# achraf-15/neural_image_compression

Hardware: AMD Instinct MI355X
Metric: images/sec (256x256 RGB, batch 32) fwd+bwd (higher is better)
Workload: dtype f32; 1 GPU; cfg2: JointAutoregressiveHierarchical(M=192,K=1) fwd+rd_loss(lambda=0.01)+bwd+Adam, 32x3x256x256 per GPU, fp32; global_batch=32, parallelism=dp1, step=eager (autograd)

## Files before the change

neural_image_compression_amd/csrc/lic_gdn.hip:

```cpp
#include "lic_common.h"
#include <stdlib.h>

namespace {

constexpr int GD_BM = 64;
constexpr int GD_BK = 16;

struct GdnParams {
  const float* x;
  const float* g;
  const float* norm;
  const float* w;
  const float* beta;
  const float* res;
  float* out;
  float* out2;
  float* cs_t;
  float* cs_dx;
  long P;
  int inverse;
};

template <int TN, int MODE>
__global__ __launch_bounds__(256) void gdn_kernel(const GdnParams p) {
  constexpr int C = 64 * TN;
  constexpr int LDX = C + 4;
  constexpr int NCH = C / GD_BK;
  constexpr int SLOTS = GD_BM * C / 4 / 256;
  __shared__ __attribute__((aligned(16))) float smem[GD_BM * LDX];
  const int tid = threadIdx.x, lane = tid & 63;
  const int wave = __builtin_amdgcn_readfirstlane(tid >> 6);
  const int wm0 = (wave >> 1) * 32, wn0 = (wave & 1) * (32 * TN);
  const int li = lane & 31, lh = lane >> 5;
  const long m0 = (long)blockIdx.x * GD_BM;
  const bool inv = p.inverse != 0;

  if (MODE == 0) {
    f32x4 a[SLOTS];
#pragma unroll
    for (int u = 0; u < SLOTS; ++u) {
      const int idx = u * 256 + tid;
      const int row = idx / (C / 4), c4 = (idx - row * (C / 4)) * 4;
      const bool ok = m0 + row < p.P;
      a[u] = *reinterpret_cast<const f32x4*>(p.x + (ok ? (m0 + row) * C + c4 : 0L));
      if (!ok) a[u] = f32x4{0.f, 0.f, 0.f, 0.f};
    }
#pragma unroll
    for (int u = 0; u < SLOTS; ++u) {
      const int idx = u * 256 + tid;
      const int row = idx / (C / 4), c4 = (idx - row * (C / 4)) * 4;
      *reinterpret_cast<f32x4*>(&smem[row * LDX + c4]) = a[u];
    }
  } else {
#pragma unroll
  for (int s0 = 0; s0 < SLOTS; s0 += 4) {
    f32x4 a[4], b[4], c[4];
    bool ok[4];
#pragma unroll
    for (int u = 0; u < 4; ++u) {
      const int idx = (s0 + u) * 256 + tid;
      const int row = idx / (C / 4), c4 = (idx - row * (C / 4)) * 4;
      ok[u] = m0 + row < p.P;
      const long off = ok[u] ? (m0 + row) * C + c4 : 0L;
      a[u] = *reinterpret_cast<const f32x4*>(p.x + off);
      b[u] = *reinterpret_cast<const f32x4*>(p.g + off);
      c[u] = *reinterpret_cast<const f32x4*>(p.norm + off);
    }
#pragma unroll
    for (int u = 0; u < 4; ++u) {
      const int idx = (s0 + u) * 256 + tid;
      const int row = idx / (C / 4), c4 = (idx - row * (C / 4)) * 4;
      f32x4 v;
#pragma unroll
      for (int e = 0; e < 4; ++e) {
        const float rs = __builtin_amdgcn_rsqf(c[u][e]);
        const float gx = b[u][e] * a[u][e];
        v[e] = inv ? 0.5f * gx * rs : -0.5f * gx * rs * (rs * rs);
      }
      if (ok[u]) *reinterpret_cast<f32x4*>(p.out2 + (m0 + row) * C + c4) = v;
      if (!ok[u]) v = f32x4{0.f, 0.f, 0.f, 0.f};
      *reinterpret_cast<f32x4*>(&smem[row * LDX + c4]) = v;
    }
  }
  }
  __syncthreads();
  if (MODE == 1 && p.cs_t && tid < C) {
    float a = 0.0f;
#pragma unroll 8
    for (int r = 0; r < GD_BM; ++r) a += smem[r * LDX + tid];
    p.cs_t[(long)blockIdx.x * C + tid] = a;
  }

  f32x16 acc[TN];
#pragma unroll
  for (int b = 0; b < TN; ++b)
#pragma unroll
    for (int r = 0; r < 16; ++r) acc[b][r] = 0.0f;
  const float* glane = p.w + ((long)(wn0 >> 5) * 512 + lane * 4);
  const float* xrow = smem + (wm0 + li) * LDX + lh * 8;
  f32x4 g0[TN][2], g1[TN][2];
  auto load_g = [&](f32x4 (&rg)[TN][2], int c) {
    const float* src = glane + (long)(c < NCH ? c : NCH - 1) * C * GD_BK;
#pragma unroll
    for (int b = 0; b < TN; ++b) {
      rg[b][0] = *reinterpret_cast<const f32x4*>(src + b * 512);
      rg[b][1] = *reinterpret_cast<const f32x4*>(src + b * 512 + 256);
    }
  };
  auto pool = [&](int c, const f32x4 (&rg)[TN][2]) {
    f32x4 a0 = *reinterpret_cast<const f32x4*>(xrow + c * GD_BK);
    f32x4 a1 = *reinterpret_cast<const f32x4*>(xrow + c * GD_BK + 4);
    if (MODE == 0) {
      a0 = a0 * a0;
      a1 = a1 * a1;
    }
#pragma unroll
    for (int t = 0; t < 8; ++t)
#pragma unroll
      for (int b = 0; b < TN; ++b)
        acc[b] = __builtin_amdgcn_mfma_f32_32x32x2f32((t < 4 ? a0 : a1)[t & 3], rg[b][t >> 2][t & 3], acc[b], 0, 0, 0);
  };
  load_g(g0, 0);
#pragma unroll 1
  for (int c = 0; c < NCH; c += 2) {
    load_g(g1, c + 1);
    pool(c, g0);
    load_g(g0, c + 2);
    pool(c + 1, g1);
  }

  __shared__ __attribute__((aligned(16))) float patch[MODE == 0 ? 4 : 1][MODE == 0 ? 1024 : 4];
  if (MODE == 1) __syncthreads();
  float* stg = MODE == 0 ? patch[wave] : smem + wave * 1024;
  const int c4 = (lane & 7) * 4, r8 = lane >> 3;
  f32x4 csum[TN];
#pragma unroll
  for (int b = 0; b < TN; ++b) csum[b] = f32x4{0.f, 0.f, 0.f, 0.f};
#pragma unroll
  for (int b = 0; b < TN; ++b) {
#pragma unroll
    for (int r = 0; r < 16; ++r) stg[((r & 3) + 8 * (r >> 2) + 4 * lh) * 32 + li] = acc[b][r];
    __builtin_amdgcn_wave_barrier();
    const int col = wn0 + b * 32 + c4;
#pragma unroll
    for (int it = 0; it < 4; ++it) {
      const int rr = it * 8 + r8;
      const long pix = m0 + wm0 + rr;
      if (pix >= p.P) continue;
      const f32x4 s4 = *reinterpret_cast<const f32x4*>(&stg[rr * 32 + c4]);
      const long off = pix * C + col;
      f32x4 o;
      if (MODE == 0) {
        const f32x4 n4 = s4 + *reinterpret_cast<const f32x4*>(p.beta + col);
        const f32x4 x4 = *reinterpret_cast<const f32x4*>(&smem[(wm0 + rr) * LDX + col]);
#pragma unroll
        for (int e = 0; e < 4; ++e)
          o[e] = x4[e] * (inv ? __builtin_amdgcn_sqrtf(n4[e]) : __builtin_amdgcn_rsqf(n4[e]));
        if (p.out2) *reinterpret_cast<f32x4*>(p.out2 + off) = n4;
        if (p.res) o += *reinterpret_cast<const f32x4*>(p.res + off);
      } else {
        const f32x4 n4 = *reinterpret_cast<const f32x4*>(p.norm + off);
        const f32x4 g4 = *reinterpret_cast<const f32x4*>(p.g + off);
        const f32x4 x4 = *reinterpret_cast<const f32x4*>(p.x + off);
#pragma unroll
        for (int e = 0; e < 4; ++e) {
          const float f = inv ? __builtin_amdgcn_sqrtf(n4[e]) : __builtin_amdgcn_rsqf(n4[e]);
          o[e] = g4[e] * f + 2.0f * x4[e] * s4[e];
        }
        csum[b] += o;
      }
      *reinterpret_cast<f32x4*>(p.out + off) = o;
    }
    __builtin_amdgcn_wave_barrier();
  }
  if (MODE == 1 && p.cs_dx) {
    __syncthreads();
    float* part = smem;
#pragma unroll
    for (int b = 0; b < TN; ++b)
      *reinterpret_cast<f32x4*>(&part[(((wave >> 1) * 8 + r8) * C) + wn0 + b * 32 + c4]) = csum[b];
    __syncthreads();
    if (tid < C) {
      float a = 0.0f;
#pragma unroll
      for (int k = 0; k < 16; ++k) a += part[k * C + tid];
      p.cs_dx[(long)blockIdx.x * C + tid] = a;
    }
  }
}

template <int TN>
__global__ __launch_bounds__(256, 2) void gdn_bwd_reg_kernel(const GdnParams p) {
  constexpr int C = 64 * TN;
  constexpr int LDX = C + 4;
  constexpr int NCH = C / GD_BK;
  __shared__ __attribute__((aligned(16))) float smem[GD_BM * LDX];
  const int tid = threadIdx.x, lane = tid & 63;
  const int wave = __builtin_amdgcn_readfirstlane(tid >> 6);
  const int wm0 = (wave >> 1) * 32, wn0 = (wave & 1) * (32 * TN);
  const int li = lane & 31, lh = lane >> 5;
  const int c4 = (lane & 7) * 4, r8 = lane >> 3;
  const long m0 = (long)blockIdx.x * GD_BM;
  const bool inv = p.inverse != 0;

  f32x4 u[TN][4], xx[TN][4];
#pragma unroll
  for (int b = 0; b < TN; ++b) {
    f32x4 gg[4], nn[4];
    bool ok[4];
#pragma unroll
    for (int it = 0; it < 4; ++it) {
      const long pix = m0 + wm0 + it * 8 + r8;
      ok[it] = pix < p.P;
      const long off = ok[it] ? pix * C + wn0 + b * 32 + c4 : 0L;
      xx[b][it] = *reinterpret_cast<const f32x4*>(p.x + off);
      gg[it] = *reinterpret_cast<const f32x4*>(p.g + off);
      nn[it] = *reinterpret_cast<const f32x4*>(p.norm + off);
    }
#pragma unroll
    for (int it = 0; it < 4; ++it) {
      const int row = wm0 + it * 8 + r8, col = wn0 + b * 32 + c4;
      f32x4 t;
#pragma unroll
      for (int e = 0; e < 4; ++e) {
        const float rs = __builtin_amdgcn_rsqf(nn[it][e]);
        const float gx = gg[it][e] * xx[b][it][e];
        t[e] = inv ? 0.5f * gx * rs : -0.5f * gx * rs * (rs * rs);
        u[b][it][e] = gg[it][e] * (inv ? __builtin_amdgcn_sqrtf(nn[it][e]) : rs);
      }
      if (ok[it]) {
        *reinterpret_cast<f32x4*>(p.out2 + (m0 + row) * C + col) = t;
      } else {
        t = f32x4{0.f, 0.f, 0.f, 0.f};
        u[b][it] = t;
        xx[b][it] = t;
      }
      *reinterpret_cast<f32x4*>(&smem[row * LDX + col]) = t;
    }
  }
  __syncthreads();
  if (p.cs_t && tid < C) {
    float a = 0.0f;
#pragma unroll 8
    for (int r = 0; r < GD_BM; ++r) a += smem[r * LDX + tid];
    p.cs_t[(long)blockIdx.x * C + tid] = a;
  }

  f32x16 acc[TN];
#pragma unroll
  for (int b = 0; b < TN; ++b)
#pragma unroll
    for (int r = 0; r < 16; ++r) acc[b][r] = 0.0f;
  const float* glane = p.w + ((long)(wn0 >> 5) * 512 + lane * 4);
  const float* xrow = smem + (wm0 + li) * LDX + lh * 8;
  f32x4 g0[TN][2], g1[TN][2];
  auto load_g = [&](f32x4 (&rg)[TN][2], int c) {
    const float* src = glane + (long)(c < NCH ? c : NCH - 1) * C * GD_BK;
#pragma unroll
    for (int b = 0; b < TN; ++b) {
      rg[b][0] = *reinterpret_cast<const f32x4*>(src + b * 512);
      rg[b][1] = *reinterpret_cast<const f32x4*>(src + b * 512 + 256);
    }
  };
  auto pool = [&](int c, const f32x4 (&rg)[TN][2]) {
    const f32x4 a0 = *reinterpret_cast<const f32x4*>(xrow + c * GD_BK);
    const f32x4 a1 = *reinterpret_cast<const f32x4*>(xrow + c * GD_BK + 4);
#pragma unroll
    for (int t = 0; t < 8; ++t)
#pragma unroll
      for (int b = 0; b < TN; ++b)
        acc[b] = __builtin_amdgcn_mfma_f32_32x32x2f32((t < 4 ? a0 : a1)[t & 3], rg[b][t >> 2][t & 3], acc[b], 0, 0, 0);
  };
  load_g(g0, 0);
#pragma unroll 1
  for (int c = 0; c < NCH; c += 2) {
    load_g(g1, c + 1);
    pool(c, g0);
    load_g(g0, c + 2);
    pool(c + 1, g1);
  }
  __syncthreads();
  float* stg = smem + wave * 1024;
  f32x4 csum[TN];
#pragma unroll
  for (int b = 0; b < TN; ++b) {
    csum[b] = f32x4{0.f, 0.f, 0.f, 0.f};
#pragma unroll
    for (int r = 0; r < 16; ++r) stg[((r & 3) + 8 * (r >> 2) + 4 * lh) * 32 + li] = acc[b][r];
    __builtin_amdgcn_wave_barrier();
#pragma unroll
    for (int it = 0; it < 4; ++it) {
      const int rr = it * 8 + r8;
      const long pix = m0 + wm0 + rr;
      if (pix >= p.P) continue;
      const f32x4 s4 = *reinterpret_cast<const f32x4*>(&stg[rr * 32 + c4]);
      f32x4 o;
#pragma unroll
      for (int e = 0; e < 4; ++e) o[e] = u[b][it][e] + 2.0f * xx[b][it][e] * s4[e];
      csum[b] += o;
      *reinterpret_cast<f32x4*>(p.out + pix * C + wn0 + b * 32 + c4) = o;
    }
    __builtin_amdgcn_wave_barrier();
  }
  if (p.cs_dx) {
    __syncthreads();
    float* part = smem;
#pragma unroll
    for (int b = 0; b < TN; ++b)
      *reinterpret_cast<f32x4*>(&part[(((wave >> 1) * 8 + r8) * C) + wn0 + b * 32 + c4]) = csum[b];
    __syncthreads();
    if (tid < C) {
      float a = 0.0f;
#pragma unroll
      for (int k = 0; k < 16; ++k) a += part[k * C + tid];
      p.cs_dx[(long)blockIdx.x * C + tid] = a;
    }
  }
}

bool gd_al16(const void* q) { return (reinterpret_cast<uintptr_t>(q) & 15) == 0; }

template <int MODE>
int gdn_launch(const GdnParams& p, int C, hipStream_t s) {
  const unsigned grid = (unsigned)cdiv64(p.P, GD_BM);
  if (C == 192)
    hipLaunchKernelGGL((gdn_kernel<3, MODE>), dim3(grid), dim3(256), 0, s, p);
  else if (C == 128)
    hipLaunchKernelGGL((gdn_kernel<2, MODE>), dim3(grid), dim3(256), 0, s, p);
  else
    hipLaunchKernelGGL((gdn_kernel<1, MODE>), dim3(grid), dim3(256), 0, s, p);
  return lic_check_launch();
}

}

LIC_EXPORT int lic_gdn_supported(int32_t C) { return C == 64 || C == 128 || C == 192; }

LIC_EXPORT int lic_gdn_fwd(const float* x, const float* gammaT_packed, const float* beta_eff, const float* res,
                           float* y, float* norm, int64_t P, int32_t C, int32_t inverse, lic_stream_t stream) {
  if (!x || !gammaT_packed || !beta_eff || !y || P <= 0) return LIC_ERR_INVALID;
  if (!lic_gdn_supported(C)) return LIC_ERR_UNSUPPORTED;
  if (!gd_al16(x) || !gd_al16(gammaT_packed) || !gd_al16(beta_eff) || !gd_al16(y) || !gd_al16(norm) || !gd_al16(res))
    return LIC_ERR_INVALID;
  if (P > 0x7FFFFFFFL * 32) return LIC_ERR_UNSUPPORTED;
  GdnParams p{x, nullptr, nullptr, gammaT_packed, beta_eff, res, y, norm, nullptr, nullptr, (long)P, inverse};
  return gdn_launch<0>(p, C, (hipStream_t)stream);
}

LIC_EXPORT int64_t lic_gdn_bwd_partial_rows(int64_t P) { return P <= 0 ? 0 : cdiv64(P, GD_BM); }

LIC_EXPORT int lic_gdn_bwd(const float* g, const float* x, const float* norm, const float* gamma_packed, float* dx,
                           float* t, float* colsum_t_partial, float* colsum_dx_partial, int64_t P, int32_t C,
                           int32_t inverse, lic_stream_t stream) {
  if (!g || !x || !norm || !gamma_packed || !dx || !t || P <= 0) return LIC_ERR_INVALID;
  if (!lic_gdn_supported(C)) return LIC_ERR_UNSUPPORTED;
  if (!gd_al16(g) || !gd_al16(x) || !gd_al16(norm) || !gd_al16(gamma_packed) || !gd_al16(dx) || !gd_al16(t))
    return LIC_ERR_INVALID;
  if (P > 0x7FFFFFFFL * 32) return LIC_ERR_UNSUPPORTED;
  GdnParams p{x, g, norm, gamma_packed, nullptr, nullptr, dx, t, colsum_t_partial, colsum_dx_partial, (long)P, inverse};
  const char* e = getenv("LIC_GDN_BWD_REG");
  if (e && e[0] == '0') return gdn_launch<1>(p, C, (hipStream_t)stream);
  const unsigned grid = (unsigned)cdiv64(p.P, GD_BM);
  hipStream_t s = (hipStream_t)stream;
  if (C == 192)
    hipLaunchKernelGGL((gdn_bwd_reg_kernel<3>), dim3(grid), dim3(256), 0, s, p);
  else if (C == 128)
    hipLaunchKernelGGL((gdn_bwd_reg_kernel<2>), dim3(grid), dim3(256), 0, s, p);
  else
    hipLaunchKernelGGL((gdn_bwd_reg_kernel<1>), dim3(grid), dim3(256), 0, s, p);
  return lic_check_launch();
}
```

neural_image_compression_amd/functional.py:

```python
from __future__ import annotations

import ctypes as C
import os
from typing import Optional, Tuple

import torch

from . import _lib as L

PEDESTAL = float(2.0 ** -36)
LIKELIHOOD_BOUND = 1e-9

PROFILE = None
PROFILE_MIN_FLOP = 0.0
FORCE_IGEMM = None
FORCE_WGRAD = None
KERNEL_TRACE = None
GRAD_VIEWS = {}
PREPARED = {}
AUX_STREAM = None


_raw_stream = getattr(torch._C, "_cuda_getCurrentRawStream", None)

# ... 368 lines not shown
        else:
            _wgrad(g, xh, dw, B=B, Hs=Ho, Ws=Wo, Cp=Cout, Hl=Hi, Wl=Wi, Cg=Cin, kh=kh, kw=kw,
                   stride=stride, pad=pad, g_is_row=True, dst_sm=taps, dst_sn=Cin * taps, dst_stap=1, job=job)
    if need_db:
        db = _bias_grad(g, B * Ho * Wo, Cout, dfr)
    return dx, dw, db


def _bias_grad(g, P, Cout, deferred=False):
    part = getattr(g, "_lic_colsum_partial", None)
    if part is not None and part.shape[1] == Cout:
        return _colsum(part, part.shape[0], Cout, deferred=deferred)
    return _colsum(g, P, Cout, deferred=deferred)


def conv2d(x, weight, bias, stride=1, padding=0, leaky=False, slope=0.01, tap_mask=0, residual=None, out=None):
    return _ConvFn.apply(x, weight, bias, stride, padding, 0, False, leaky, slope, tap_mask, residual, out)


class _JoinChannelsFn(torch.autograd.Function):

    @staticmethod
    def forward(ctx, a, b, buf):
        ca, cb = a.shape[1], b.shape[1]
        if buf.shape[-1] != ca + cb or a.data_ptr() != buf.data_ptr() or \
                b.data_ptr() != buf.data_ptr() + buf.element_size() * ca:
            raise ValueError("join_channels: the operands are not the two channel ranges of the buffer")
        ctx.ca = ca
        return _nchw_view(buf)

    @staticmethod
    def backward(ctx, g):
        return g[:, :ctx.ca], g[:, ctx.ca:], None


def join_channels(a, b, buf):
    return _JoinChannelsFn.apply(a, b, buf)


def pack_conv_weight(weight: torch.Tensor) -> torch.Tensor:
    _require_cuda(weight)
    return _pack_conv_weight(weight.detach(), False, for_dgrad=False)


@torch.no_grad()
def conv2d_prepacked(x, w_packed, bias, cout, kernel, stride=1, padding=0, leaky=False, slope=0.01, tap_mask=0,
                     pin_tile=False):
    _require_cuda(x, w_packed, bias)
    xh = _nhwc(x)
    B, Hi, Wi, Cin = xh.shape
    Ho, Wo = conv_out_size(Hi, Wi, kernel, stride, padding, False)
    out = torch.empty((B, Ho, Wo, cout), device=x.device, dtype=torch.float32)
    global FORCE_IGEMM
    saved = FORCE_IGEMM
    if pin_tile and Cin % 4 == 0 and cout % 64 == 0:
        FORCE_IGEMM = (64, 1, 0)
    try:
        _igemm(xh, w_packed, out, B=B, Hi=Hi, Wi=Wi, Cin=Cin, Ho=Ho, Wo=Wo, Cout=cout, kh=kernel, kw=kernel,
               stride=stride, pad=padding, transposed=False, bias=bias,
               epilogue=L.EPI_LEAKY if leaky else L.EPI_NONE, slope=slope, tap_mask=tap_mask)
    finally:
        FORCE_IGEMM = saved
    return _nchw_view(out)


def conv_transpose2d(x, weight, bias, stride=1, padding=0, output_padding=0, leaky=False, slope=0.01,
                     residual=None):
    return _ConvFn.apply(x, weight, bias, stride, padding, output_padding, True, leaky, slope, 0, residual)


def _kpad(kh, kw, c):
    return (kh * kw * c + 3) // 4 * 4


def _image_conv_columns(xh, weight, stride, pad):
    B, Hi, Wi, Cin = xh.shape
    Cout, _, kh, kw = weight.shape
    Ho, Wo = conv_out_size(Hi, Wi, kh, stride, pad, False)
    Kp = _kpad(kh, kw, Cin)
    P = B * Ho * Wo
    col = torch.empty((P, Kp), device=xh.device, dtype=torch.float32)
    L.check(L.load().lic_im2col(_ptr(xh), _ptr(col), B, Hi, Wi, Cin, Ho, Wo, kh, kw, stride, pad, Kp,
                                _stream()), "lic_im2col")
    taps = kh * kw
    wpk = prepared(weight, "f32.stem")
    if wpk is None:
        wp = torch.zeros((Kp, Cout), device=xh.device, dtype=torch.float32)
        _permute3(weight.contiguous(), wp, (taps, Cin, Cout), (1, taps, Cin * taps), (Cin * Cout, Cout, 1))
        wpk = _pack_dense(wp)
    return col, wpk, Ho, Wo, Kp


def _image_conv_backward(col, weight, g, stride, pad, in_shape, need_dx, need_dw, need_db):
    B, Hi, Wi, Cin = in_shape
    _, Ho, Wo, Cout = g.shape
    _, _, kh, kw = weight.shape
    taps, Kp, P = kh * kw, col.shape[1], B * Ho * Wo
    lib = L.load()
    dx = dw = db = None
    if need_dx:
        wpT = torch.zeros((Cout, Kp), device=g.device, dtype=torch.float32)
        _permute3(weight.contiguous(), wpT, (Cout, Cin, taps), (Cin * taps, taps, 1), (Kp, 1, Cin))
        dcol = torch.empty((P, Kp), device=g.device, dtype=torch.float32)
        _igemm(g, _pack_dense(wpT), dcol, B=1, Hi=1, Wi=P, Cin=Cout, Ho=1, Wo=P, Cout=Kp, kh=1, kw=1, stride=1,
               pad=0, transposed=False)
        dxh = torch.empty((B, Hi, Wi, Cin), device=g.device, dtype=torch.float32)
        L.check(lib.lic_col2im(_ptr(dcol), None, _ptr(dxh), B, Ho, Wo, Cin, Hi, Wi, kh, kw, stride,
                               pad, Kp, _stream()), "lic_col2im")
        dx = _nchw_view(dxh)
    dfr = DEFER_FP32 and (need_dw or need_db) and can_defer(weight)
    if need_dw:
        dw = grad_like(weight)
        if dfr:
            job = L.ReduceJob()
            _wgrad(col, g, dw, B=1, Hs=1, Ws=P, Cp=Kp, Hl=1, Wl=P, Cg=Cout, kh=1, kw=1, stride=1, pad=0,
                   g_is_row=False, dst_sm=Cout, dst_sn=1, dst_stap=0, job=job)
            job.mdiv, job.sm, job.smr, job.sn, job.Mvalid = Cin, 1, taps, Cin * taps, taps * Cin
        else:
            tmp = torch.empty((Kp, Cout), device=g.device, dtype=torch.float32)
            _wgrad(col, g, tmp, B=1, Hs=1, Ws=P, Cp=Kp, Hl=1, Wl=P, Cg=Cout, kh=1, kw=1, stride=1, pad=0,
                   g_is_row=False, dst_sm=Cout, dst_sn=1, dst_stap=0)
            _permute3(tmp, dw, (taps, Cin, Cout), (Cin * Cout, Cout, 1), (1, taps, Cin * taps))
    if need_db:
        db = _bias_grad(g, P, Cout, dfr)
    return dx, dw, db


class _ImageConvFn(torch.autograd.Function):

    @staticmethod
    def forward(ctx, x, weight, bias, stride, pad, leaky, slope):
        _require_cuda(x, weight, bias)
        xh = _nhwc(x)
        B = xh.shape[0]
        Cout = weight.shape[0]
        col, wp, Ho, Wo, Kp = _image_conv_columns(xh, weight, stride, pad)
        P = B * Ho * Wo
        out = torch.empty((B, Ho, Wo, Cout), device=x.device, dtype=torch.float32)
        _igemm(col, wp, out, B=1, Hi=1, Wi=P, Cin=Kp, Ho=1, Wo=P, Cout=Cout, kh=1, kw=1, stride=1,
               pad=0, transposed=False, bias=bias, epilogue=L.EPI_LEAKY if leaky else L.EPI_NONE,
               slope=slope)
        ctx.save_for_backward(col, weight, out if leaky else None)
        ctx.cfg = (stride, pad, leaky, slope, tuple(xh.shape), bias is not None)
        return _nchw_view(out)

    @staticmethod
    def backward(ctx, gy):
        col, weight, yh = ctx.saved_tensors
        stride, pad, leaky, slope, in_shape, has_bias = ctx.cfg
        g = _nhwc(gy)
        if leaky:
            g = _leaky_bwd(yh, g, slope)
        elif hasattr(gy, "_lic_colsum_partial"):
            g._lic_colsum_partial = gy._lic_colsum_partial
        dx, dw, db = _image_conv_backward(col, weight, g, stride, pad, in_shape, ctx.needs_input_grad[0],
                                          ctx.needs_input_grad[1], has_bias and ctx.needs_input_grad[2])
        return dx, dw, db, None, None, None, None


class _ImageConvGDNFn(torch.autograd.Function):

    @staticmethod
    def forward(ctx, x, weight, bias, beta, gamma, stride, pad, inverse, beta_bound, gamma_bound, pedestal, keep=True):
        _require_cuda(x, weight, bias, beta, gamma)
        xh = _nhwc(x)
        B = xh.shape[0]
        Cout = weight.shape[0]
        col, wp, Ho, Wo, Kp = _image_conv_columns(xh, weight, stride, pad)
        P = B * Ho * Wo
        beta_e, gT = _gdn_operands(beta, gamma, beta_bound, gamma_bound, pedestal)
        y = torch.empty((B, Ho, Wo, Cout), device=x.device, dtype=torch.float32)
        conv_out = torch.empty_like(y) if keep else None
        norm = torch.empty_like(y) if keep else None
        _igemm(col, wp, y, B=1, Hi=1, Wi=P, Cin=Kp, Ho=1, Wo=P, Cout=Cout, kh=1, kw=1, stride=1,
               pad=0, transposed=False, bias=bias, epilogue=L.EPI_CONV_IGDN if inverse else L.EPI_CONV_GDN,
               out2=norm, out3=conv_out, aux=gT, aux2=beta_e)
        ctx.save_for_backward(col, weight, conv_out, norm, beta, gamma)
        ctx.cfg = (stride, pad, tuple(xh.shape), inverse, beta_bound, gamma_bound, bias is not None, pedestal)
        return _nchw_view(y)

    @staticmethod
    def backward(ctx, gy):
        col, weight, conv_out, norm, beta, gamma = ctx.saved_tensors
        stride, pad, in_shape, inverse, beta_bound, gamma_bound, has_bias, pedestal = ctx.cfg
        need = ctx.needs_input_grad
        g_conv, dbeta, dgamma = _gdn_backward(conv_out, norm, beta, gamma, _nhwc(gy), inverse,
                                              beta_bound, gamma_bound, pedestal, True, need[3], need[4])
        dx, dw, db = _image_conv_backward(col, weight, g_conv, stride, pad, in_shape, need[0], need[1],
                                          has_bias and need[2])
        return dx, dw, db, dbeta, dgamma, None, None, None, None, None, None, None


class _ImageConvTFn(torch.autograd.Function):

    @staticmethod
    def forward(ctx, x, weight, bias, stride, pad, out_pad):
        _require_cuda(x, weight, bias)
        xh = _nhwc(x)
        B, Hi, Wi, Cin = xh.shape
        _, Cout, kh, kw = weight.shape
        Ho, Wo = conv_out_size(Hi, Wi, kh, stride, pad, True, out_pad)
        taps, Kp, P = kh * kw, _kpad(kh, kw, Cout), B * Hi * Wi
        lib = L.load()
        wpk = prepared(weight, "f32.head")
        if wpk is None:
            wp = torch.zeros((Cin, Kp), device=x.device, dtype=torch.float32)
            _permute3(weight.contiguous(), wp, (Cin, Cout, taps), (Cout * taps, taps, 1), (Kp, 1, Cout))
            wpk = _pack_dense(wp)
        col = torch.empty((P, Kp), device=x.device, dtype=torch.float32)
        _igemm(xh, wpk, col, B=1, Hi=1, Wi=P, Cin=Cin, Ho=1, Wo=P, Cout=Kp, kh=1, kw=1, stride=1, pad=0,
               transposed=False)
        out = torch.empty((B, Ho, Wo, Cout), device=x.device, dtype=torch.float32)
        L.check(lib.lic_col2im(_ptr(col), _ptr(bias), _ptr(out), B, Hi, Wi, Cout, Ho, Wo, kh, kw, stride,
                               pad, Kp, _stream()), "lic_col2im")
        ctx.save_for_backward(xh, weight)
        ctx.cfg = (stride, pad, (Ho, Wo), bias is not None)
        return _nchw_view(out)

    @staticmethod
    def backward(ctx, gy):
        xh, weight = ctx.saved_tensors
        stride, pad, (Ho, Wo), has_bias = ctx.cfg
        g = _nhwc(gy)
        B, Hi, Wi, Cin = xh.shape
        _, Cout, kh, kw = weight.shape
        taps, Kp, P = kh * kw, _kpad(kh, kw, Cout), B * Hi * Wi
        lib = L.load()
        dcol = torch.empty((P, Kp), device=g.device, dtype=torch.float32)
        L.check(lib.lic_im2col(_ptr(g), _ptr(dcol), B, Ho, Wo, Cout, Hi, Wi, kh, kw, stride, pad, Kp,
                               _stream()), "lic_im2col")
        dx = dw = db = None
        if ctx.needs_input_grad[0]:
            wpk = prepared(weight, "f32.head_dx")
            if wpk is None:
                wpT = torch.zeros((Kp, Cin), device=g.device, dtype=torch.float32)
                _permute3(weight.contiguous(), wpT, (taps, Cout, Cin), (1, taps, Cout * taps),
                          (Cout * Cin, Cin, 1))
                wpk = _pack_dense(wpT)
            dxh = torch.empty_like(xh)
            _igemm(dcol, wpk, dxh, B=1, Hi=1, Wi=P, Cin=Kp, Ho=1, Wo=P, Cout=Cin, kh=1, kw=1, stride=1,
                   pad=0, transposed=False)
            dx = _nchw_view(dxh)
        dfr = DEFER_FP32 and (ctx.needs_input_grad[1] or (has_bias and ctx.needs_input_grad[2])) and can_defer(weight)
        if ctx.needs_input_grad[1]:
            dw = grad_like(weight)
            if dfr:
                job = L.ReduceJob()
                _wgrad(xh, dcol, dw, B=1, Hs=1, Ws=P, Cp=Cin, Hl=1, Wl=P, Cg=Kp, kh=1, kw=1, stride=1, pad=0,
                       g_is_row=True, dst_sm=1, dst_sn=Kp, dst_stap=0, job=job)
                job.mdiv, job.sm, job.smr, job.sn, job.Mvalid = Cout, 1, taps, Cout * taps, taps * Cout
            else:
                tmp = torch.empty((Cin, Kp), device=g.device, dtype=torch.float32)
                _wgrad(xh, dcol, tmp, B=1, Hs=1, Ws=P, Cp=Cin, Hl=1, Wl=P, Cg=Kp, kh=1, kw=1, stride=1, pad=0,
                       g_is_row=True, dst_sm=1, dst_sn=Kp, dst_stap=0)
                _permute3(tmp, dw, (Cin, taps, Cout), (Kp, Cout, 1), (Cout * taps, 1, taps))
        if has_bias and ctx.needs_input_grad[2]:
            db = _colsum(g, B * Ho * Wo, Cout, deferred=dfr)
        return dx, dw, db, None, None, None


def image_conv2d(x, weight, bias, stride, padding, leaky=False, slope=0.01):
    return _ImageConvFn.apply(x, weight, bias, stride, padding, leaky, slope)


def image_conv_transpose2d(x, weight, bias, stride, padding, output_padding):
    return _ImageConvTFn.apply(x, weight, bias, stride, padding, output_padding)


class _LeakyFn(torch.autograd.Function):
    @staticmethod
    def forward(ctx, x, slope):
        _require_cuda(x)
        xc = x.contiguous()
        y = _leaky_bwd(xc, xc, slope)
        ctx.save_for_backward(y)
        ctx.slope = slope
        return y

    @staticmethod
    def backward(ctx, gy):
        (y,) = ctx.saved_tensors
        return _leaky_bwd(y, gy.contiguous(), ctx.slope), None


def leaky_relu(x, slope=0.01):
    return _LeakyFn.apply(x, slope)


class _GDNFn(torch.autograd.Function):
    @staticmethod
    def forward(ctx, x, beta, gamma, inverse, beta_bound, gamma_bound, pedestal, res, keep=True):
        _require_cuda(x, beta, gamma, res)
        lib = L.load()
        xh = _nhwc(x)
        B, H, W, Cc = xh.shape
        beta_e, gT = _gdn_operands(beta, gamma, beta_bound, gamma_bound, pedestal)
        out = torch.empty_like(xh)
        norm = torch.empty_like(xh) if keep else None
        resh = None if res is None else _nhwc(res)
        P = B * H * W
        if lib.lic_gdn_supported(Cc):
            if KERNEL_TRACE is not None:
                KERNEL_TRACE.add(f"gdn_kernel<{Cc // 64}, {int(inverse)}>")
            _timed(f"gdn_kernel<{Cc // 64}, 0>", 2 * P * Cc * Cc, 4 * 3 * P * Cc,
                   lambda: L.check(lib.lic_gdn_fwd(_ptr(xh), _ptr(gT), _ptr(beta_e), _ptr(resh), _ptr(out), _ptr(norm),
                                                   P, Cc, int(inverse), _stream()), "lic_gdn_fwd"))
        else:
            _igemm(xh, gT, out, B=1, Hi=1, Wi=P, Cin=Cc, Ho=1, Wo=P, Cout=Cc, kh=1, kw=1, stride=1, pad=0,
                   transposed=False, bias=beta_e, prologue=1, epilogue=L.EPI_IGDN if inverse else L.EPI_GDN,
                   out2=norm, aux=xh, res=resh)
        ctx.save_for_backward(xh, norm, beta, gamma)
        ctx.cfg = (inverse, beta_bound, gamma_bound, res is not None, pedestal)
        return _nchw_view(out)

    @staticmethod
    def backward(ctx, gy):
        xh, norm, beta, gamma = ctx.saved_tensors
        inverse, beta_bound, gamma_bound, has_res, pedestal = ctx.cfg
        dxh, dbeta, dgamma = _gdn_backward(xh, norm, beta, gamma, _nhwc(gy), inverse, beta_bound,
                                           gamma_bound, pedestal, *ctx.needs_input_grad[:3])
        dres = gy if has_res else None
        dx = None if dxh is None else _nchw_view(dxh)
        if dx is not None and hasattr(dxh, "_lic_colsum_partial"):
            dx._lic_colsum_partial = dxh._lic_colsum_partial
        return dx, dbeta, dgamma, None, None, None, None, dres, None


def _gdn_operands(beta, gamma, beta_bound, gamma_bound, pedestal):
    beta_e, gT = prepared(beta, "f32.beta_e"), prepared(gamma, "f32.gdn_gT")
    if beta_e is None or gT is None:
        Cc = beta.numel()
        _, _, beta_e, gamma_e = _gdn_reparam(beta, gamma, beta_bound, gamma_bound, pedestal)
        gT = _pack(gamma_e, 1, Cc, Cc, 0, 1, Cc)
    return beta_e, gT


def _gdn_gamma_packed(gamma, gamma_bound, pedestal):
    gp = prepared(gamma, "f32.gdn_g")
    if gp is None:
        lib = L.load()
        gamma_c = gamma.contiguous()
        gamma_e = torch.empty_like(gamma_c)
        L.check(lib.lic_gdn_reparam(_ptr(gamma_c), _ptr(gamma_e), gamma_c.numel(), gamma_bound, pedestal, _stream()),
                "lic_gdn_reparam")
        gp = _pack_dense(gamma_e)
    return gp


def _gdn_reparam(beta, gamma, beta_bound, gamma_bound, pedestal):
    lib = L.load()
    Cc = beta.numel()
    beta_c, gamma_c = beta.contiguous(), gamma.contiguous()
    beta_e = torch.empty_like(beta_c)
    gamma_e = torch.empty_like(gamma_c)
    L.check(lib.lic_gdn_reparam(_ptr(beta_c), _ptr(beta_e), Cc, beta_bound, pedestal, _stream()),
            "lic_gdn_reparam")
    L.check(lib.lic_gdn_reparam(_ptr(gamma_c), _ptr(gamma_e), Cc * Cc, gamma_bound, pedestal,
                                _stream()), "lic_gdn_reparam")
    return beta_c, gamma_c, beta_e, gamma_e


def _gdn_backward(xh, norm, beta, gamma, g, inverse, beta_bound, gamma_bound, pedestal, need_dx, need_dbeta,
                  need_dgamma):
    lib = L.load()
    B, H, W, Cc = xh.shape
    P = B * H * W
    t = torch.empty_like(xh)
    dxh = dbeta = dgamma = None
    cs_dx = None
    dbe = None
    beta_c, gamma_c = beta.contiguous(), gamma.contiguous()
    gp = _gdn_gamma_packed(gamma, gamma_bound, pedestal) if need_dx else None
    dfr = DEFER_FP32 and (need_dbeta or need_dgamma) and \
        can_defer(beta if need_dbeta else None, gamma if need_dgamma else None)
    dbeta_d = None
    if need_dx and lib.lic_gdn_supported(Cc):
        dxh = torch.empty_like(xh)
        rows = lib.lic_gdn_bwd_partial_rows(P)
        pt = torch.empty((rows, Cc), device=xh.device, dtype=torch.float32)
        pdx = torch.empty((rows, Cc), device=xh.device, dtype=torch.float32)
        if KERNEL_TRACE is not None:
            KERNEL_TRACE.add(f"gdn_bwd_kernel<{Cc // 64}, {int(inverse)}>")
        _timed(f"gdn_bwd_reg_kernel<{Cc // 64}>", 2 * P * Cc * Cc, 4 * 5 * P * Cc,
               lambda: L.check(lib.lic_gdn_bwd(_ptr(g), _ptr(xh), _ptr(norm), _ptr(gp), _ptr(dxh), _ptr(t), _ptr(pt),
                                               _ptr(pdx), P, Cc, int(inverse), _stream()), "lic_gdn_bwd"))
        if need_dbeta:
            if dfr:
                dbeta_d = _colsum(pt, rows, Cc, deferred=True, reparam=(beta_c, beta_bound)).view(beta_c.shape)
            else:
                dbe = _colsum(pt, rows, Cc)
        cs_dx = pdx
    elif need_dx and Cc % 4 == 0:
        dxh = torch.empty_like(xh)
        _igemm(g, gp, dxh, B=1, Hi=1, Wi=P, Cin=Cc, Ho=1, Wo=P, Cout=Cc, kh=1, kw=1, stride=1,
               pad=0, transposed=False, prologue=3 if inverse else 2,
               epilogue=L.EPI_IGDN_BWD if inverse else L.EPI_GDN_BWD, aux=g, aux2=xh, aux3=norm, out2=t)
    else:
        L.check(lib.lic_gdn_dnorm(_ptr(g), _ptr(xh), _ptr(norm), _ptr(t), xh.numel(), int(inverse),
                                  _stream()), "lic_gdn_dnorm")
        if need_dx:
            dxh = torch.empty_like(xh)
            _igemm(t, gp, dxh, B=1, Hi=1, Wi=P, Cin=Cc, Ho=1, Wo=P, Cout=Cc, kh=1, kw=1,
                   stride=1, pad=0, transposed=False, epilogue=L.EPI_IGDN_BWD if inverse else L.EPI_GDN_BWD,
                   aux=g, aux2=xh, aux3=norm)
    dge = None
    if dfr:
        dbeta, dgamma = dbeta_d, None
        if need_dbeta and dbeta is None:
            dbeta = _colsum(t, P, Cc, deferred=True, reparam=(beta_c, beta_bound)).view(beta_c.shape)
        if need_dgamma:
            dgamma = torch.empty_like(gamma_c)
            job = L.ReduceJob()
            _wgrad(t, xh, dgamma, B=1, Hs=1, Ws=P, Cp=Cc, Hl=1, Wl=P, Cg=Cc, kh=1, kw=1, stride=1, pad=0,
                   g_is_row=False, dst_sm=Cc, dst_sn=1, dst_stap=0, sq_g=1, job=job)
            job.epilogue, job.param, job.bound = L.REDUCE_EPI_REPARAM, gamma_c.data_ptr(), gamma_bound
            _PENDING_KEEP.append(gamma_c)
        if cs_dx is not None and dxh is not None:
            dxh._lic_colsum_partial = cs_dx
        return dxh, dbeta, dgamma
    if need_dbeta and dbe is None:
        dbe = _colsum(t, P, Cc)
    if need_dgamma:
        dge = torch.empty_like(gamma_c)
        _wgrad(t, xh, dge, B=1, Hs=1, Ws=P, Cp=Cc, Hl=1, Wl=P, Cg=Cc, kh=1, kw=1, stride=1, pad=0,
               g_is_row=False, dst_sm=Cc, dst_sn=1, dst_stap=0, sq_g=1)
    dbeta, dgamma = _reparam_bwd2(beta_c if need_dbeta else None, dbe, beta_bound,
                                  gamma_c if need_dgamma else None, dge, gamma_bound)
    if cs_dx is not None and dxh is not None:
        dxh._lic_colsum_partial = cs_dx
    return dxh, dbeta, dgamma


class _ConvGDNFn(torch.autograd.Function):

    @staticmethod
    def forward(ctx, x, weight, bias, beta, gamma, stride, pad, out_pad, transposed, inverse, beta_bound,
                gamma_bound, pedestal, keep=True):
        _require_cuda(x, weight, bias, beta, gamma)
        xh = _nhwc(x)
        B, Hi, Wi, Cin = xh.shape
        kh, kw = weight.shape[2], weight.shape[3]
        Cout = weight.shape[1] if transposed else weight.shape[0]
        Ho, Wo = conv_out_size(Hi, Wi, kh, stride, pad, transposed, out_pad)
        wp = _pack_conv_weight(weight, transposed, for_dgrad=False)
        beta_e, gT = _gdn_operands(beta, gamma, beta_bound, gamma_bound, pedestal)
        y = torch.empty((B, Ho, Wo, Cout), device=x.device, dtype=torch.float32)
        conv_out = torch.empty_like(y) if keep else None
        norm = torch.empty_like(y) if keep else None
        _igemm(xh, wp, y, B=B, Hi=Hi, Wi=Wi, Cin=Cin, Ho=Ho, Wo=Wo, Cout=Cout, kh=kh, kw=kw, stride=stride,
               pad=pad, transposed=transposed, bias=bias,
               epilogue=L.EPI_CONV_IGDN if inverse else L.EPI_CONV_GDN, out2=norm, out3=conv_out, aux=gT,
               aux2=beta_e)
        ctx.save_for_backward(xh, weight, conv_out, norm, beta, gamma)
        ctx.cfg = (stride, pad, transposed, inverse, beta_bound, gamma_bound, bias is not None, pedestal)
        return _nchw_view(y)

    @staticmethod
    def backward(ctx, gy):
        xh, weight, conv_out, norm, beta, gamma = ctx.saved_tensors
        stride, pad, transposed, inverse, beta_bound, gamma_bound, has_bias, pedestal = ctx.cfg
        need = ctx.needs_input_grad
        g_conv, dbeta, dgamma = _gdn_backward(conv_out, norm, beta, gamma, _nhwc(gy), inverse,
                                              beta_bound, gamma_bound, pedestal, True, need[3], need[4])
        dx, dw, db = _conv_backward(xh, weight, g_conv, stride, pad, transposed, 0, need[0], need[1],
                                    has_bias and need[2])
        return dx, dw, db, dbeta, dgamma, None, None, None, None, None, None, None, None, None


def will_backprop(*ts) -> bool:
    return torch.is_grad_enabled() and any(t is not None and t.requires_grad for t in ts)


def fused_gdn_supported(cin: int, cout: int) -> bool:
    return bool(L.load().lic_igemm_fused_gdn_supported(int(cin), int(cout)))


def fused_gdn_preferred(x_shape, weight_shape, stride, padding, transposed, output_padding=0) -> bool:
    B, Cin, Hi, Wi = x_shape
    kh, kw = weight_shape[2], weight_shape[3]
    Cout = weight_shape[1] if transposed else weight_shape[0]
    Ho, Wo = conv_out_size(Hi, Wi, kh, stride, padding, transposed, output_padding)
    d = L.IgemmDesc()
    if not transposed and Cin < 4:
        d.B, d.Hi, d.Wi, d.Cin, d.Ho, d.Wo, d.Cout = 1, 1, B * Ho * Wo, _kpad(kh, kw, Cin), 1, B * Ho * Wo, Cout
        d.kh = d.kw = d.stride = 1
        d.pad = d.transposed = 0
    else:
        d.B, d.Hi, d.Wi, d.Cin, d.Ho, d.Wo, d.Cout = B, Hi, Wi, Cin, Ho, Wo, Cout
        d.kh, d.kw, d.stride, d.pad, d.transposed = kh, kw, stride, padding, int(transposed)
    d.in_ld, d.out_ld, d.out2_ld, d.out3_ld = d.Cin, Cout, Cout, Cout
    return bool(L.load().lic_igemm_fused_gdn_preferred(C.byref(d)))


def conv_gdn(x, weight, bias, beta, gamma, stride, padding, inverse, beta_bound, gamma_bound, pedestal=PEDESTAL,
             transposed=False, output_padding=0):
    if not transposed and weight.shape[1] < 4:
        return _ImageConvGDNFn.apply(x, weight, bias, beta, gamma, stride, padding, bool(inverse),
                                     float(beta_bound), float(gamma_bound), float(pedestal),
                                     will_backprop(x, weight, bias, beta, gamma))
    return _ConvGDNFn.apply(x, weight, bias, beta, gamma, stride, padding, output_padding, bool(transposed),
                            bool(inverse), float(beta_bound), float(gamma_bound), float(pedestal),
                            will_backprop(x, weight, bias, beta, gamma))


def gdn(x, beta, gamma, inverse, beta_bound, gamma_bound, pedestal=PEDESTAL, residual=None):
    return _GDNFn.apply(x, beta, gamma, bool(inverse), float(beta_bound), float(gamma_bound),
                        float(pedestal), residual, will_backprop(x, beta, gamma, residual))


_QUANT_CASTS = [None, None]


class _QuantizeFn(torch.autograd.Function):
    @staticmethod
    def forward(ctx, v, u, training, cast_in=False, cast_out=False):
        _require_cuda(v, u)
        vh = _nhwc(v)
        uh = None if u is None else _nhwc(u)
        out = torch.empty_like(vh)
        _QUANT_CASTS[0] = _QUANT_CASTS[1] = None
        if (cast_in or cast_out) and vh.numel() % 4 == 0:
            v16 = torch.empty_like(vh, dtype=torch.bfloat16) if cast_in else None
            o16 = torch.empty_like(vh, dtype=torch.bfloat16) if cast_out else None
            L.check(L.load().lic_quantize_bf16(_ptr(vh), _ptr(uh), _ptr(out), _ptr(v16), _ptr(o16), vh.numel(),
                                               int(training), _stream()), "lic_quantize_bf16")
            _QUANT_CASTS[0], _QUANT_CASTS[1] = v16, o16
        else:
            L.check(L.load().lic_quantize(_ptr(vh), _ptr(uh), _ptr(out), vh.numel(), int(training), _stream()),
                    "lic_quantize")
        ctx.training = training
        return _nchw_view(out)

    @staticmethod
    def backward(ctx, g):
        return (g if ctx.training else torch.zeros_like(g)), None, None, None, None


def attach_bf16(t: torch.Tensor, t16_nhwc: Optional[torch.Tensor]):
    if t16_nhwc is not None:
        t._lic_bf16 = (t._version, t16_nhwc)


def quantize(v, u=None, training=True, cast_in=False, cast_out=False):
    if not (cast_in or cast_out):
        return _QuantizeFn.apply(v, u, training)
    res = _QuantizeFn.apply(v, u, training, cast_in, cast_out)
    attach_bf16(v, _QUANT_CASTS[0])
    attach_bf16(res, _QUANT_CASTS[1])
    _QUANT_CASTS[0] = _QUANT_CASTS[1] = None
    return res


class _EntropyParamsActFn(torch.autograd.Function):

    @staticmethod
    def forward(ctx, raw, M, K):
        _require_cuda(raw)
        rh = _nhwc(raw)
        B, H, W, CH = rh.shape
        out = torch.empty_like(rh)
        L.check(L.load().lic_entropy_params_fwd(_ptr(rh), _ptr(out), B * H * W, M, K, _stream()),
                "lic_entropy_params_fwd")
        ctx.save_for_backward(rh, out)
        ctx.cfg = (M, K)
        return _nchw_view(out)

    @staticmethod
    def backward(ctx, g):
        rh, out = ctx.saved_tensors
        M, K = ctx.cfg
        gh = _nhwc(g)
        B, H, W, CH = rh.shape
        d = torch.empty_like(rh)
        L.check(L.load().lic_entropy_params_bwd(_ptr(rh), _ptr(out), _ptr(gh), _ptr(d), B * H * W, M, K,
                                                _stream()), "lic_entropy_params_bwd")
        return _nchw_view(d), None, None


def entropy_params_activation(raw, M, K):
    return _EntropyParamsActFn.apply(raw, M, K)


class _GmmLikelihoodFn(torch.autograd.Function):

    @staticmethod
    def forward(ctx, x, params, K, bound):
        _require_cuda(x, params)
        ctx.set_materialize_grads(False)
        xh, ph = _nhwc(x), _nhwc(params)
        B, H, W, M = xh.shape
        p = torch.empty_like(xh)
        logp = torch.empty_like(xh)
        L.check(L.load().lic_gmm_likelihood_fwd(_ptr(xh), _ptr(ph), _ptr(p), _ptr(logp), B * H * W, M, K,
                                                bound, _stream()), "lic_gmm_likelihood_fwd")
        ctx.save_for_backward(xh, ph)
        ctx.cfg = (K, bound)
        return _nchw_view(p), _nchw_view(logp)

    @staticmethod
    def backward(ctx, gp, glogp):
        xh, ph = ctx.saved_tensors
        K, bound = ctx.cfg
        B, H, W, M = xh.shape
        gph = None if gp is None else _nhwc(gp)
        glh = None if glogp is None else _nhwc(glogp)
        dx = torch.empty_like(xh)
        dpar = torch.empty_like(ph)
# ... 169 lines not shown
```

Measured before the change: 1438 images/s.

## Add persistent warp-specialized GDN forward kernel with producer/consumer pipelining

Adds a persistent GDN forward kernel, launched with one block per CU, where four producer waves stream x tiles into double-buffered LDS with buffer loads and write the epilogue outputs. The other four waves run the squared-x by gamma MFMA GEMM. This overlaps global memory traffic with the matrix math across tiles instead of running them in sequence inside each block. It becomes the default path, with an env var to fall back to the old kernel. The cost is a large LDS footprint, heavy barrier coordination, and GDN forward being only one part of the whole training step.

```diff
diff --git a/neural_image_compression_amd/csrc/lic_gdn.hip b/neural_image_compression_amd/csrc/lic_gdn.hip
--- a/neural_image_compression_amd/csrc/lic_gdn.hip
+++ b/neural_image_compression_amd/csrc/lic_gdn.hip
@@ -318,7 +318,165 @@
   }
 }
 
+constexpr int GP_THREADS = 512;
+
+__device__ __forceinline__ void gp_barrier() { asm volatile("s_waitcnt lgkmcnt(0)\n\ts_barrier" ::: "memory"); }
+
+template <int TN, bool RES>
+__global__ __launch_bounds__(GP_THREADS) void gdn_pipe_fwd_kernel(const GdnParams p) {
+  constexpr int C = 64 * TN;
+  constexpr int LDX = C + 4;
+  constexpr int NCH = C / GD_BK;
+  constexpr int MS = 16 * C / 4 / 64;
+  __shared__ __attribute__((aligned(16))) float lds[2 * GD_BM * LDX + GD_BM * C + C];
+  float* const sb = lds + 2 * GD_BM * LDX;
+  float* const bs = sb + GD_BM * C;
+  const int tid = threadIdx.x, lane = tid & 63;
+  const int wave = __builtin_amdgcn_readfirstlane(tid >> 6);
+  const long T = (p.P + GD_BM - 1) / GD_BM;
+  const int n = (int)((T - blockIdx.x + gridDim.x - 1) / gridDim.x);
+  const bool inv = p.inverse != 0;
+
+  if (wave >= 4) {
+    const int mw = wave - 4;
+    auto row = [&](int u) { return mw * 16 + (u * 64 + lane) / (C / 4); };
+    auto c4 = [&](int u) { return ((u * 64 + lane) % (C / 4)) * 4; };
+    auto go = [&](int u) { return (int)((row(u) * C + c4(u)) * 4); };
+    auto rsrc = [&](const float* base, long tile) {
+      const long vr = base ? p.P - tile * GD_BM : 0;
+      const unsigned bytes = (unsigned)((vr < GD_BM ? vr : GD_BM) * C * 4);
+      return __builtin_amdgcn_make_buffer_rsrc(const_cast<float*>(base + tile * GD_BM * C), 0, (int)bytes, 0x00020000);
+    };
+    typedef unsigned u32x4 __attribute__((ext_vector_type(4)));
+    if (tid - 256 < C / 4) *reinterpret_cast<f32x4*>(&bs[(tid - 256) * 4]) = *reinterpret_cast<const f32x4*>(p.beta + (tid - 256) * 4);
+    f32x4 a[MS];
+    auto load = [&](long tile) {
+      const __amdgpu_buffer_rsrc_t rs = rsrc(p.x, tile);
+#pragma unroll
+      for (int u = 0; u < MS; ++u) a[u] = __builtin_bit_cast(f32x4, __builtin_amdgcn_raw_buffer_load_b128(rs, go(u), 0, 0));
+    };
+    auto put = [&](float* xb) {
+#pragma unroll
+      for (int u = 0; u < MS; ++u) *reinterpret_cast<f32x4*>(&xb[row(u) * LDX + c4(u)]) = a[u];
+    };
+    auto finish = [&](long tile, const float* xb) {
+      const __amdgpu_buffer_rsrc_t ry = rsrc(p.out, tile), rn = rsrc(p.out2, tile), rr = rsrc(p.res, tile);
+#pragma unroll
+      for (int u = 0; u < MS; ++u) {
+        const f32x4 n4 = *reinterpret_cast<const f32x4*>(&sb[row(u) * C + c4(u)]) +
+                         *reinterpret_cast<const f32x4*>(&bs[c4(u)]);
+        const f32x4 x4 = *reinterpret_cast<const f32x4*>(&xb[row(u) * LDX + c4(u)]);
+        f32x4 o;
+#pragma unroll
+        for (int e = 0; e < 4; ++e)
+          o[e] = x4[e] * (inv ? __builtin_amdgcn_sqrtf(n4[e]) : __builtin_amdgcn_rsqf(n4[e]));
+        __builtin_amdgcn_raw_buffer_store_b128(__builtin_bit_cast(u32x4, n4), rn, go(u), 0, 0);
+        if (RES) o += __builtin_bit_cast(f32x4, __builtin_amdgcn_raw_buffer_load_b128(rr, go(u), 0, 0));
+        __builtin_amdgcn_raw_buffer_store_b128(__builtin_bit_cast(u32x4, o), ry, go(u), 0, 0);
+        if ((u & 3) == 3) __builtin_amdgcn_sched_barrier(0);
+      }
+    };
+    auto xbuf = [&](int k) { return lds + (k & 1) * GD_BM * LDX; };
+    auto tile = [&](int k) { return blockIdx.x + (long)k * gridDim.x; };
+    load(tile(0));
+    put(xbuf(0));
+    gp_barrier();
+    if (n > 1) {
+      load(tile(1));
+      put(xbuf(1));
+    }
+    gp_barrier();
+    gp_barrier();
+#pragma unroll 1
+    for (int k = 1; k + 1 < n; ++k) {
+      if (RES) finish(tile(k - 1), xbuf(k + 1));
+      load(tile(k + 1));
+      if (!RES) finish(tile(k - 1), xbuf(k + 1));
+      put(xbuf(k + 1));
+      gp_barrier();
+      gp_barrier();
+    }
+    if (n > 1) {
+      finish(tile(n - 2), xbuf(n));
+      gp_barrier();
+      gp_barrier();
+    }
+    finish(tile(n - 1), xbuf(n - 1));
+  } else {
+    const int wm0 = (wave >> 1) * 32, wn0 = (wave & 1) * (32 * TN);
+    const int li = lane & 31, lh = lane >> 5;
+    const float* glane = p.w + ((long)(wn0 >> 5) * 512 + lane * 4);
+    f32x4 gr[3][TN][2];
+    auto load_g = [&](f32x4 (&rg)[TN][2], int c) {
+      const float* src = glane + (long)c * C * GD_BK;
+#pragma unroll
+      for (int b = 0; b < TN; ++b) {
+        rg[b][0] = *reinterpret_cast<const f32x4*>(src + b * 512);
+        rg[b][1] = *reinterpret_cast<const f32x4*>(src + b * 512 + 256);
+      }
+    };
+    load_g(gr[0], 0);
+    load_g(gr[1], 1);
+    gp_barrier();
+#pragma unroll 1
+    for (int k = 0; k < n; ++k) {
+      const float* xrow = lds + (k & 1) * GD_BM * LDX + (wm0 + li) * LDX + lh * 8;
+      f32x16 acc[TN];
+#pragma unroll
+      for (int b = 0; b < TN; ++b)
+#pragma unroll
+        for (int r = 0; r < 16; ++r) acc[b][r] = 0.0f;
+      f32x4 xa[2][2];
+      xa[0][0] = *reinterpret_cast<const f32x4*>(xrow);
+      xa[0][1] = *reinterpret_cast<const f32x4*>(xrow + 4);
+#pragma unroll
+      for (int c = 0; c < NCH; ++c) {
+        if (c + 2 < NCH) load_g(gr[(c + 2) % 3], c + 2);
+        if (c + 1 < NCH) {
+          xa[(c + 1) & 1][0] = *reinterpret_cast<const f32x4*>(xrow + (c + 1) * GD_BK);
+          xa[(c + 1) & 1][1] = *reinterpret_cast<const f32x4*>(xrow + (c + 1) * GD_BK + 4);
+        }
+        const f32x4 a0 = xa[c & 1][0] * xa[c & 1][0];
+        const f32x4 a1 = xa[c & 1][1] * xa[c & 1][1];
+#pragma unroll
+        for (int t = 0; t < 8; ++t)
+#pragma unroll
+          for (int b = 0; b < TN; ++b)
+            acc[b] = __builtin_amdgcn_mfma_f32_32x32x2f32((t < 4 ? a0 : a1)[t & 3], gr[c % 3][b][t >> 2][t & 3], acc[b], 0,
+                                                          0, 0);
+        __builtin_amdgcn_sched_barrier(0);
+      }
+      load_g(gr[0], 0);
+      load_g(gr[1], 1);
+      gp_barrier();
+#pragma unroll
+      for (int b = 0; b < TN; ++b)
+#pragma unroll
+        for (int r = 0; r < 16; ++r) sb[(wm0 + (r & 3) + 8 * (r >> 2) + 4 * lh) * C + wn0 + b * 32 + li] = acc[b][r];
+      gp_barrier();
+    }
+  }
+}
+
 bool gd_al16(const void* q) { return (reinterpret_cast<uintptr_t>(q) & 15) == 0; }
+
+int gd_pipe() {
+  const char* e = getenv("LIC_GDN_PIPE");
+  return !(e && e[0] == '0');
+}
+
+unsigned gd_pipe_grid(long P) {
+  static int ncu[64] = {0};
+  int dev = 0;
+  if (hipGetDevice(&dev) != hipSuccess || dev < 0 || dev >= 64) dev = 0;
+  if (ncu[dev] <= 0) {
+    int v = 0;
+    if (hipDeviceGetAttribute(&v, hipDeviceAttributeMultiprocessorCount, dev) != hipSuccess || v <= 0) v = 256;
+    ncu[dev] = v;
+  }
+  const long T = cdiv64(P, GD_BM);
+  return (unsigned)(T < ncu[dev] ? T : ncu[dev]);
+}
 
 template <int MODE>
 int gdn_launch(const GdnParams& p, int C, hipStream_t s) {
@@ -344,7 +502,17 @@
     return LIC_ERR_INVALID;
   if (P > 0x7FFFFFFFL * 32) return LIC_ERR_UNSUPPORTED;
   GdnParams p{x, nullptr, nullptr, gammaT_packed, beta_eff, res, y, norm, nullptr, nullptr, (long)P, inverse};
-  return gdn_launch<0>(p, C, (hipStream_t)stream);
+  if (!gd_pipe()) return gdn_launch<0>(p, C, (hipStream_t)stream);
+  const unsigned grid = gd_pipe_grid(p.P);
+  hipStream_t s = (hipStream_t)stream;
+  const bool r = res != nullptr;
+  if (C == 192)
+    hipLaunchKernelGGL((r ? gdn_pipe_fwd_kernel<3, true> : gdn_pipe_fwd_kernel<3, false>), dim3(grid), dim3(GP_THREADS), 0, s, p);
+  else if (C == 128)
+    hipLaunchKernelGGL((r ? gdn_pipe_fwd_kernel<2, true> : gdn_pipe_fwd_kernel<2, false>), dim3(grid), dim3(GP_THREADS), 0, s, p);
+  else
+    hipLaunchKernelGGL((r ? gdn_pipe_fwd_kernel<1, true> : gdn_pipe_fwd_kernel<1, false>), dim3(grid), dim3(GP_THREADS), 0, s, p);
+  return lic_check_launch();
 }
 
 LIC_EXPORT int64_t lic_gdn_bwd_partial_rows(int64_t P) { return P <= 0 ? 0 : cdiv64(P, GD_BM); }
diff --git a/neural_image_compression_amd/functional.py b/neural_image_compression_amd/functional.py
--- a/neural_image_compression_amd/functional.py
+++ b/neural_image_compression_amd/functional.py
@@ -694,7 +694,10 @@
         if lib.lic_gdn_supported(Cc):
             if KERNEL_TRACE is not None:
                 KERNEL_TRACE.add(f"gdn_kernel<{Cc // 64}, {int(inverse)}>")
-            _timed(f"gdn_kernel<{Cc // 64}, 0>", 2 * P * Cc * Cc, 4 * 3 * P * Cc,
+            pipe = os.environ.get("LIC_GDN_PIPE", "1")[:1] != "0"
+            name = f"gdn_pipe_fwd_kernel<{Cc // 64}, {str(res is not None).lower()}>" if pipe else \
+                f"gdn_kernel<{Cc // 64}, 0>"
+            _timed(name, 2 * P * Cc * Cc, 4 * 3 * P * Cc,
                    lambda: L.check(lib.lic_gdn_fwd(_ptr(xh), _ptr(gT), _ptr(beta_e), _ptr(resh), _ptr(out), _ptr(norm),
                                                    P, Cc, int(inverse), _stream()), "lic_gdn_fwd"))
         else:
```

New measurement: 1442 images/s (median of 6 runs). Within noise of the previous version (+0.2%).
